# slbouknight/accelerated-ray-tracer

Hardware: AMD Instinct MI355X
Metric: Mrays/s, 1200x800 random scene @ 500 spp (frame ms in ms_per_step) (higher is better)
Workload: dtype f32

## Files before the change

accelerated-ray-tracer_amd/csrc/rt_device_funcs.h:

```cpp
#pragma once
#include <hip/hip_runtime.h>
#include <float.h>
#include <stdint.h>

#include "../../include/rt_abi.h"
#include "rt_device.h"
#include "rt_xorwow.h"

#define DEV __device__ __forceinline__

namespace {

struct f3 { float x, y, z; };
DEV f3 mk3(float x, float y, float z) { f3 r; r.x = x; r.y = y; r.z = z; return r; }
DEV f3 ld3(const float* p) { return mk3(p[0], p[1], p[2]); }
DEV f3 operator+(f3 a, f3 b) { return mk3(a.x + b.x, a.y + b.y, a.z + b.z); }
DEV f3 operator-(f3 a, f3 b) { return mk3(a.x - b.x, a.y - b.y, a.z - b.z); }
DEV f3 operator*(f3 a, f3 b) { return mk3(a.x * b.x, a.y * b.y, a.z * b.z); }
DEV f3 operator*(float t, f3 v) { return mk3(t * v.x, t * v.y, t * v.z); }
DEV f3 operator-(f3 a) { return mk3(-a.x, -a.y, -a.z); }
DEV f3 sdiv(f3 v, float t) { return mk3(v.x / t, v.y / t, v.z / t); }
DEV float dot(f3 a, f3 b) { return fmaf(a.z, b.z, fmaf(a.x, b.x, a.y * b.y)); }
DEV f3 cross(f3 a, f3 b) { return mk3(fmaf(a.y, b.z, -(a.z * b.y)), -fmaf(a.x, b.z, -(a.z * b.x)), fmaf(a.x, b.y, -(a.y * b.x))); }
DEV float length(f3 v) { return sqrtf(fmaf(v.z, v.z, fmaf(v.x, v.x, v.y * v.y))); }
// ... 212 lines not shown
    float t0 = (lo_skip.x - o.x) * inv.x, t1 = (hi_prim.x - o.x) * inv.x;
    if (inv.x < 0.0f) { const float tmp = t0; t0 = t1; t1 = tmp; }
    tmin = t0 > tmin ? t0 : tmin;
    tmax = t1 < tmax ? t1 : tmax;
    t0 = (lo_skip.y - o.y) * inv.y; t1 = (hi_prim.y - o.y) * inv.y;
    if (inv.y < 0.0f) { const float tmp = t0; t0 = t1; t1 = tmp; }
    tmin = t0 > tmin ? t0 : tmin;
    tmax = t1 < tmax ? t1 : tmax;
    t0 = (lo_skip.z - o.z) * inv.z; t1 = (hi_prim.z - o.z) * inv.z;
    if (inv.z < 0.0f) { const float tmp = t0; t0 = t1; t1 = tmp; }
    tmin = t0 > tmin ? t0 : tmin;
    tmax = t1 < tmax ? t1 : tmax;
    return !(tmax <= tmin);
}

DEV void sphere_uv(f3 p, float& u, float& v) {
    const float PI_F = 3.141592654f;
    const float theta = cr_acos(-p.y);
    const float phi = cr_atan2(-p.z, p.x) + PI_F;
    u = phi / (2 * PI_F);
    v = theta / PI_F;
}

template <bool SPHERES_ONLY, bool NEED_UV>
DEV HitRec resolve_hit(const SceneView& sc, const Ray& r, const HitInfo& h) {
    HitRec rec;
    rec.u = 0.f; rec.v = 0.f;
    const int kind = SPHERES_ONLY ? RT_PRIM_SPHERE : RT_PRIM_KIND(h.prim);
    const int idx = RT_PRIM_INDEX(h.prim);
    if (!SPHERES_ONLY && kind == RT_PRIM_MEDIUM) {
        rec.p = ray_at(r, h.t);
        rec.n = mk3(1, 0, 0);
        rec.mat = sc.media[idx].mat;
        return rec;
    }
    Ray q = r;
    rt_instance in;
    const bool through_instance = !SPHERES_ONLY && h.inst >= 0;
    if (through_instance) { in = sc.instances[h.inst]; q = to_object_space(in, r); }
    if (kind == RT_PRIM_SPHERE) {
        const rt_sphere s = sc.spheres[idx];
        const f3 cc = fma3(q.tm, ld3(s.vel), ld3(s.c0));
        rec.p = ray_at(q, h.t);
        rec.n = sdiv(rec.p - cc, s.radius);
        if (NEED_UV && sc.materials[s.mat].pad != 0.0f) sphere_uv(rec.n, rec.u, rec.v);
        rec.mat = s.mat;
    } else {
        const rt_quad qd = sc.quads[idx];
        const f3 P = ray_at(q, h.t);
        const f3 pl = P - ld3(qd.Q);
        const f3 w = ld3(qd.w);
        rec.u = dot(w, cross(pl, ld3(qd.v)));
        rec.v = dot(w, cross(ld3(qd.u), pl));
        f3 n = ld3(qd.n);
        if (dot(n, q.d) > 0.f) n = -n;
        rec.p = P; rec.n = n; rec.mat = qd.mat;
    }
    if (through_instance) {
        if (in.flags & RT_INST_ROTATE_Y) {
            const float c = in.cos_t, s = in.sin_t;
            const float px = fmaf(c, rec.p.x, s * rec.p.z);
            const float pz = fmaf(c, rec.p.z, -(s * rec.p.x));
            const float nx = fmaf(c, rec.n.x, s * rec.n.z);
            const float nz = fmaf(c, rec.n.z, -(s * rec.n.x));
            rec.p = mk3(px, rec.p.y, pz);
            rec.n = unit_vector(mk3(nx, rec.n.y, nz));
            f3 dir_seen = r.d;
            if (dot(rec.n, dir_seen) > 0.f) rec.n = -rec.n;
        }
        if (in.flags & RT_INST_TRANSLATE) rec.p = rec.p + ld3(in.offset);
    }
    return rec;
}

DEV uint32_t wanghash(uint32_t x) {
    x = (x ^ 61u) ^ (x >> 16); x *= 9u; x = x ^ (x >> 4); x *= 0x27d4eb2du; x = x ^ (x >> 15); return x;
}
DEV float u2m11(uint32_t h) { return fmaf((float)((h >> 8) & 0x00FFFFFFu), (1.0f / 8388607.5f), -1.0f); }
DEV f3 perlin_grad(int xi, int yi, int zi) {
    const uint32_t h = wanghash((uint32_t)xi * 73856093u ^ (uint32_t)yi * 19349663u ^ (uint32_t)zi * 83492791u);
    return unit_vector(mk3(u2m11(h), u2m11(wanghash(h)), u2m11(wanghash(h ^ 0x9e3779b9u))));
}
DEV float perlin_noise(f3 p) {
    const float fx = floorf(p.x), fy = floorf(p.y), fz = floorf(p.z);
    const float u = p.x - fx, v = p.y - fy, w = p.z - fz;
    const int i = (int)fx, j = (int)fy, k = (int)fz;
    const float uu = u * u * (3.0f - 2.0f * u), vv = v * v * (3.0f - 2.0f * v), ww = w * w * (3.0f - 2.0f * w);
    float accum = 0.0f;
#pragma unroll
    for (int a = 0; a < 2; ++a)
#pragma unroll
        for (int b = 0; b < 2; ++b)
#pragma unroll
            for (int c = 0; c < 2; ++c) {
                const f3 g = perlin_grad(i + a, j + b, k + c);
                const f3 weight = mk3(u - (float)a, v - (float)b, w - (float)c);
                const float s = (a ? uu : (1.0f - uu)) * (b ? vv : (1.0f - vv)) * (c ? ww : (1.0f - ww));
                accum = fmaf(s, dot(g, weight), accum);
            }
    return accum;
}
__device__ __attribute__((noinline)) float perlin_turb(f3 p, int depth) {
    float accum = 0.0f, weight = 1.0f;
    f3 temp = p;
    for (int i = 0; i < depth; ++i) {
        accum = fmaf(weight, perlin_noise(temp), accum);
        weight *= 0.5f;
        temp = mk3(temp.x * 2.0f, temp.y * 2.0f, temp.z * 2.0f);
    }
    return fabsf(accum);
}

DEV float clamp01(float x) { return x < 0 ? 0 : (x > 1 ? 1 : x); }
template <int TEX>
DEV f3 texture_value(const SceneView& sc, int tex, float u, float v, f3 p) {
    rt_texture t = sc.textures[tex];
    while (t.kind == RT_TEX_CHECKER || (TEX >= 2 && t.kind == RT_TEX_UV_OFFSET)) {
        if (TEX >= 2 && t.kind == RT_TEX_UV_OFFSET) {
            float uu = u + t.scale; uu -= floorf(uu);
            float vv = v + t.p[0]; vv = fminf(fmaxf(vv, 0.f), 1.f);
            u = uu; v = vv;
            t = sc.textures[t.a];
        } else {
            const int xi = (int)floorf(t.scale * p.x);
            const int yi = (int)floorf(t.scale * p.y);
            const int zi = (int)floorf(t.scale * p.z);
            const bool is_even = ((xi + yi + zi) & 1) == 0;
            t = sc.textures[is_even ? t.a : t.b];
        }
    }
    if (TEX < 2 || t.kind == RT_TEX_SOLID) return ld3(t.color);
    if (t.kind == RT_TEX_IMAGE) {
        if (t.a < 0 || t.b <= 0 || t.c <= 0) return mk3(0, 1, 1);
        u = clamp01(u); v = clamp01(v);
        int i = (int)(u * (float)t.b); if (i > t.b - 1) i = t.b - 1;
        int j = (int)((1.f - v) * (float)t.c); if (j > t.c - 1) j = t.c - 1;
        const uint8_t* px = sc.images + (size_t)t.a + (size_t)(j * t.b + i) * 3;
        const float inv255 = 1.f / 255.f;
        return mk3(inv255 * (float)px[0], inv255 * (float)px[1], inv255 * (float)px[2]);
    }
    if (t.kind == RT_TEX_NOODLE) {
        const f3 dir = mk3(t.p[3], t.p[4], t.p[5]);
        const float uu = dot(p, dir);
        const float wig = perlin_turb(t.p[7] * p, t.a);
        const float stripes = fabsf(cr_sin(fmaf(t.scale, uu, t.p[6] * wig)));
        const float q = clamp01((stripes - 0.75f) / (0.98f - 0.75f));
        const float w = q * q * (3.0f - 2.0f * q);
        return fma3(1.f - w, mk3(t.p[0], t.p[1], t.p[2]), w * ld3(t.color));
    }
    if (t.kind == RT_TEX_FELT) {
        const float m = perlin_noise(t.scale * p);
        const float phase = fmaf(p.x, t.p[1], 2.0f * perlin_turb(0.5f * p, 2));
        const float fibers = 0.5f * (1.0f + cr_sin(phase));
        float gain = fmaf(t.p[2], fibers - 0.5f, fmaf(t.p[0], m - 0.5f, 1.0f));
        gain = fminf(fmaxf(gain, 0.7f), 1.2f);
        return gain * ld3(t.color);
    }
    const float s = cr_sin(fmaf(t.scale, p.z, 10.0f * perlin_turb(p, 7)));
    const float g = 0.5f * (1.0f + s);
    return mk3(g, g, g);
}

DEV f3 random_in_unit_sphere(rt_xorwow& g) {
    for (;;) {
        const float a = 2.0f * rt_xorwow_uniform(g) - 1.0f;
        const float b = 2.0f * rt_xorwow_uniform(g) - 1.0f;
        const float c = 2.0f * rt_xorwow_uniform(g) - 1.0f;
        const f3 p = mk3(a, b, c);
        if (dot(p, p) < 1.0f) return p;
    }
}
DEV f3 reflect(f3 v, f3 n) { return fma3(-(2.0f * dot(v, n)), n, v); }
DEV bool refract(f3 v, f3 n, float ni_over_nt, f3& refracted) {
    const f3 uv = unit_vector(v);
    const float dt = dot(uv, n);
    const float disc = fmaf(-(ni_over_nt * ni_over_nt), fmaf(-dt, dt, 1.0f), 1.0f);
    if (disc > 0.0f) {
        refracted = fma3(-sqrtf(disc), n, ni_over_nt * fma3(-dt, n, uv));
        return true;
    }
    return false;
}
DEV float schlick(float cosine, float ref_idx) {
    float r0 = (1.0f - ref_idx) / (1.0f + ref_idx);
    r0 = r0 * r0;
    return fmaf(1.0f - r0, cr_pow5(1.0f - cosine), r0);
}

DEV f3 dielectric_direction(f3 d_in, f3 n, float ior, rt_xorwow& g) {
    f3 outward_normal;
    const f3 reflected = reflect(d_in, n);
    float ni_over_nt, cosine, reflect_prob;
    f3 refracted = mk3(0.f, 0.f, 0.f);
    const float d_n = dot(d_in, n);
    if (d_n > 0.0f) {
        outward_normal = -n;
        ni_over_nt = ior;
        cosine = d_n / length(d_in);
        cosine = sqrtf(fmaxf(0.0f, fmaf(-(ior * ior), fmaf(-cosine, cosine, 1.0f), 1.0f)));
    } else {
        outward_normal = n;
        ni_over_nt = 1.0f / ior;
        cosine = -d_n / length(d_in);
    }
    if (refract(d_in, outward_normal, ni_over_nt, refracted)) reflect_prob = schlick(cosine, ior);
    else reflect_prob = 1.0f;
    return (rt_xorwow_uniform(g) < reflect_prob) ? reflected : refracted;
}

template <int TEX>
DEV bool shade(const SceneView& sc, const Ray& in, const HitRec& rec, rt_xorwow& g, f3& emitted, f3& attenuation, Ray& out) {
    const rt_material m = sc.materials[rec.mat];
    emitted = mk3(0.f, 0.f, 0.f);
    out.o = rec.p;
    out.tm = in.tm;
    switch (m.kind) {
    case RT_MAT_LAMBERTIAN: {
        const f3 target = (rec.p + rec.n) + random_in_unit_sphere(g);
        out.d = target - rec.p;
        attenuation = (TEX > 0 && m.tex >= 0) ? texture_value<TEX>(sc, m.tex, rec.u, rec.v, rec.p) : ld3(m.albedo);
        return true;
    }
    case RT_MAT_METAL: {
        const f3 reflected = reflect(unit_vector(in.d), rec.n);
        const f3 rs = random_in_unit_sphere(g);
        out.d = fma3(m.fuzz, rs, reflected);
        attenuation = ld3(m.albedo);
        return dot(out.d, rec.n) > 0.0f;
    }
    case RT_MAT_DIELECTRIC: {
        attenuation = mk3(1.0f, 1.0f, 1.0f);
        out.d = dielectric_direction(in.d, rec.n, m.ior, g);
        return true;
    }
    case RT_MAT_DIFFUSE_LIGHT: {
        emitted = (TEX > 0 && m.tex >= 0) ? texture_value<TEX>(sc, m.tex, rec.u, rec.v, rec.p) : ld3(m.albedo);
        return false;
    }
    default: {
        out.d = random_in_unit_sphere(g);
        attenuation = (TEX > 0 && m.tex >= 0) ? texture_value<TEX>(sc, m.tex, rec.u, rec.v, rec.p) : ld3(m.albedo);
        return true;
    }
    }
}

DEV Ray camera_get_ray(const rt_camera& c, float s, float t, rt_xorwow& g) {
    f3 p;
    do {
        const float a = rt_xorwow_uniform(g);
        const float b = rt_xorwow_uniform(g);
        p = 2.0f * mk3(a, b, 0.0f) - mk3(1.0f, 1.0f, 0.0f);
    } while (dot(p, p) >= 1.0f);
    const f3 rd = c.lens_radius * p;
    const f3 cu = ld3(c.u), cv = ld3(c.v);
    const f3 offset = fma3(rd.x, cu, rd.y * cv);
    const double tm = fma((double)rt_xorwow_uniform(g), c.time1 - c.time0, c.time0);
    const f3 origin = ld3(c.origin);
    Ray r;
    r.o = origin + offset;
    r.d = (fma3(t, ld3(c.vertical), fma3(s, ld3(c.horizontal), ld3(c.lower_left_corner))) - origin) - offset;
    r.tm = (float)tm;
    return r;
}

DEV float apply_gamma(float c, float gamma) {
    if (gamma == 1.0f) return c;
    const float inv = 1.0f / gamma;
    return cr_pow(fmaxf(c, 0.0f), inv);
}

template <typename P>
DEV f3 miss_color(const P& fp, const Ray& r) {
    f3 bg = mk3(fp.background[0], fp.background[1], fp.background[2]);
    if (fp.use_gradient_bg) {
        const f3 ud = unit_vector(r.d);
        const float t = 0.5f * (ud.y + 1.0f);
        bg = mk3(fmaf(t, 0.5f, 1.0f - t), fmaf(t, 0.7f, 1.0f - t), (1.0f - t) + t);
    }
    return bg;
}

DEV bool work_to_pixel(const rt_frame_params& fp, uint32_t w, int& i, int& lrow) {
    const uint32_t tile = fp.tile_order ? fp.tile_order[w >> 6] : (w >> 6), within = w & 63u;
    const uint32_t tx = tile % (uint32_t)fp.tiles_x, ty = tile / (uint32_t)fp.tiles_x;
    i = (int)(tx * 8u + (within & 7u));
    lrow = (int)(ty * 8u + (within >> 3));
    return i < fp.nx && lrow < fp.local_rows;
}
DEV int local_to_global_row(const rt_frame_params& fp, int lrow) {
    const int t = lrow / fp.tile_rows;
    return (fp.tile_first + t * fp.tile_stride) * fp.tile_rows + (lrow - t * fp.tile_rows);
}

DEV void store_pixel(const rt_frame_params& fp, int i, int lrow, f3 col) {
    const float k = (float)(1.0 / (double)(float)fp.ns);
    col = mk3(col.x * k, col.y * k, col.z * k);
    float* px = fp.fb + ((size_t)lrow * fp.nx + i) * 3;
    px[0] = apply_gamma(col.x, fp.gamma);
    px[1] = apply_gamma(col.y, fp.gamma);
    px[2] = apply_gamma(col.z, fp.gamma);
}

template <int LDS_MODE>
DEV SceneView stage_scene(const rt_scene_dev& sd, unsigned char* lds) {
    SceneView v;
    v.nodes = sd.nodes; v.spheres = sd.spheres; v.quads = sd.quads; v.boxes = sd.boxes; v.instances = sd.instances;
    v.media = sd.media; v.materials = sd.materials; v.textures = sd.textures; v.images = sd.images; v.n_nodes = sd.n_nodes;
    if (LDS_MODE >= 1 && LDS_MODE <= 3) {
        float4* dst = reinterpret_cast<float4*>(lds);
        const float4* src = reinterpret_cast<const float4*>(sd.nodes);
        const int n16 = sd.n_nodes * 2;
        for (int k = threadIdx.x; k < n16; k += blockDim.x) dst[k] = src[k];
        v.nodes = reinterpret_cast<const rt_node*>(lds);
        if (LDS_MODE >= 2) {
            float4* dst2 = dst + n16;
            const float4* src2 = reinterpret_cast<const float4*>(sd.spheres);
            const int m16 = sd.n_spheres * 2;
            for (int k = threadIdx.x; k < m16; k += blockDim.x) dst2[k] = src2[k];
            v.spheres = reinterpret_cast<const rt_sphere*>(dst2);
            if (LDS_MODE >= 3) {
                float4* dst3 = dst2 + m16;
                const float4* src3 = reinterpret_cast<const float4*>(sd.materials);
                const int q16 = sd.n_materials * 2;
                for (int k = threadIdx.x; k < q16; k += blockDim.x) dst3[k] = src3[k];
                v.materials = reinterpret_cast<const rt_material*>(dst3);
                float4* dst4 = dst3 + q16;
                const float4* src4 = reinterpret_cast<const float4*>(sd.textures);
                const int r16 = sd.n_textures * 4;
                for (int k = threadIdx.x; k < r16; k += blockDim.x) dst4[k] = src4[k];
                v.textures = reinterpret_cast<const rt_texture*>(dst4);
            }
        }
        __syncthreads();
    }
    return v;
}

template <bool SPHERES_ONLY>
DEV bool trace(const SceneView& sc, const Ray& r, HitInfo& best, unsigned int* pass_count = nullptr) {
    const f3 inv = mk3(1.0f / r.d.x, 1.0f / r.d.y, 1.0f / r.d.z);
    const float tmin = 0.001f;
    best.t = FLT_MAX; best.prim = -1; best.inst = -1;
    const float4* nodes4 = reinterpret_cast<const float4*>(sc.nodes);
    int i = 0;
    const int n = sc.n_nodes;
    while (i < n) {
        const float4 a = nodes4[2 * i], b = nodes4[2 * i + 1];
        int next = RT_NODE_SKIP(__float_as_int(a.w));
        if (slab_test(a, b, r.o, inv, tmin, best.t)) {
            if (pass_count) atomicAdd(&pass_count[i], 1u);
            const int32_t prim = __float_as_int(b.w);
            if (prim >= 0) leaf_test<SPHERES_ONLY>(sc, prim, r, tmin, best);
            else next = i + 1;
        }
        i = next;
    }
    return best.prim >= 0;
}

DEV bool inv_is_finite(const f3 inv) {
    return fabsf(inv.x) < INFINITY && fabsf(inv.y) < INFINITY && fabsf(inv.z) < INFINITY;
}

DEV void slab_interval(const float4 lo_skip, const float4 hi_prim, const f3 o, const f3 inv, float tmin, float& t_enter, float& t_exit) {
    float tmax = FLT_MAX;
    float t0 = (lo_skip.x - o.x) * inv.x, t1 = (hi_prim.x - o.x) * inv.x;
    if (inv.x < 0.0f) { const float tmp = t0; t0 = t1; t1 = tmp; }
    tmin = t0 > tmin ? t0 : tmin;
    tmax = t1 < tmax ? t1 : tmax;
    t0 = (lo_skip.y - o.y) * inv.y; t1 = (hi_prim.y - o.y) * inv.y;
    if (inv.y < 0.0f) { const float tmp = t0; t0 = t1; t1 = tmp; }
    tmin = t0 > tmin ? t0 : tmin;
    tmax = t1 < tmax ? t1 : tmax;
    t0 = (lo_skip.z - o.z) * inv.z; t1 = (hi_prim.z - o.z) * inv.z;
    if (inv.z < 0.0f) { const float tmp = t0; t0 = t1; t1 = tmp; }
    tmin = t0 > tmin ? t0 : tmin;
    tmax = t1 < tmax ? t1 : tmax;
    t_enter = tmin; t_exit = tmax;
}

DEV bool lane_not(bool b) { return __builtin_amdgcn_inverse_ballot_w64(~__builtin_amdgcn_ballot_w64(b)); }

DEV bool slab_interval_open(float tmin, float tmax, float x0, float x1, float y0, float y1, float z0, float z1) {
    float lo = __builtin_amdgcn_fmed3f(tmin, x0, x1), hi = __builtin_amdgcn_fmed3f(tmax, x0, x1);
    lo = __builtin_amdgcn_fmed3f(lo, y0, y1); hi = __builtin_amdgcn_fmed3f(hi, y0, y1);
    lo = __builtin_amdgcn_fmed3f(lo, z0, z1); hi = __builtin_amdgcn_fmed3f(hi, z0, z1);
    return !(hi <= lo);
}

DEV bool slab_test_finite(const float4 lo_skip, const float4 hi_prim, const f3 o, const f3 inv, float tmin, float tmax) {
    const float x0 = (lo_skip.x - o.x) * inv.x, x1 = (hi_prim.x - o.x) * inv.x;
    const float y0 = (lo_skip.y - o.y) * inv.y, y1 = (hi_prim.y - o.y) * inv.y;
    const float z0 = (lo_skip.z - o.z) * inv.z, z1 = (hi_prim.z - o.z) * inv.z;
    return slab_interval_open(tmin, tmax, x0, x1, y0, y1, z0, z1);
}

struct LooseRay { f3 clo, chi; };
DEV bool loose_ok(const f3 inv, const f3 o, const float* bound) {
    const float ex = fabsf(inv.x) * (fabsf(o.x) + bound[0]), ey = fabsf(inv.y) * (fabsf(o.y) + bound[1]), ez = fabsf(inv.z) * (fabsf(o.z) + bound[2]);
    return fmaxf(fmaxf(ex, ey), ez) < 1e30f;
}
DEV LooseRay loose_setup(const f3 inv, const f3 o, const float* bound) {
    const float k = 9.5367431640625e-07f;
    const float ex = k * (fabsf(inv.x) * (fabsf(o.x) + bound[0])), ey = k * (fabsf(inv.y) * (fabsf(o.y) + bound[1])), ez = k * (fabsf(inv.z) * (fabsf(o.z) + bound[2]));
    const float cx = -(o.x * inv.x), cy = -(o.y * inv.y), cz = -(o.z * inv.z);
    LooseRay r;
    r.clo = mk3(inv.x < 0.0f ? cx + ex : cx - ex, inv.y < 0.0f ? cy + ey : cy - ey, inv.z < 0.0f ? cz + ez : cz - ez);
    r.chi = mk3(inv.x < 0.0f ? cx - ex : cx + ex, inv.y < 0.0f ? cy - ey : cy + ey, inv.z < 0.0f ? cz - ez : cz + ez);
    return r;
}
DEV bool slab_test_loose(const float4 lo_skip, const float4 hi_prim, const f3 inv, const LooseRay& lr, float tmin, float tmax) {
    const float x0 = fmaf(lo_skip.x, inv.x, lr.clo.x), x1 = fmaf(hi_prim.x, inv.x, lr.chi.x);
    const float y0 = fmaf(lo_skip.y, inv.y, lr.clo.y), y1 = fmaf(hi_prim.y, inv.y, lr.chi.y);
    const float z0 = fmaf(lo_skip.z, inv.z, lr.clo.z), z1 = fmaf(hi_prim.z, inv.z, lr.chi.z);
    return slab_interval_open(tmin, tmax, x0, x1, y0, y1, z0, z1);
}

}
```

accelerated-ray-tracer_amd/csrc/rt_kernel_staged.h:

```cpp
#pragma once
#ifndef RT_STEP_UNROLL
#define RT_STEP_UNROLL 2
#endif
#include "rt_device_funcs.h"
#include "rt_launch.h"

#ifdef RT_DIAG
#define DIAG_ADD(slot, value) do { const unsigned long long v_ = (unsigned long long)(value); if ((threadIdx.x & 63) == 0) diag_local[slot] += v_; } while (0)
#define DIAG_T(slot) do { const unsigned long long n_ = __builtin_readcyclecounter(); diag_time[slot] += n_ - diag_t_last; diag_t_last = n_; } while (0)
#else
#define DIAG_ADD(slot, value) do { } while (0)
#define DIAG_T(slot) do { } while (0)
#endif

template <bool SPHERES_ONLY, int TEX, bool NEED_UV, int LDS_MODE>
__global__ void __launch_bounds__((SPHERES_ONLY && TEX < 2) ? RT_LEAN_MAX_THREADS : RT_HEAVY_MAX_THREADS, (SPHERES_ONLY && TEX < 2) ? RT_LEAN_MIN_WAVES : RT_HEAVY_MIN_WAVES) rt_render_staged_kernel(rt_scene_dev sd, rt_frame_params fp) {
    extern __shared__ __attribute__((aligned(16))) unsigned char lds[];
#ifdef RT_DIAG
    unsigned long long diag_local[16] = {0, 0, 0, 0, 0, 0, 0, 0, 0, 0, 0, 0, 0, 0, 0, 0};
    unsigned long long diag_time[8] = {0, 0, 0, 0, 0, 0, 0, 0};
    unsigned long long diag_shade_cycles = 0;
    unsigned long long diag_t_last = 0;
    const unsigned long long diag_t_start = __builtin_amdgcn_s_memrealtime();
    if ((threadIdx.x & 63) == 0) atomicMin(fp.ray_counter + RT_DIAG_T0_SLOT, diag_t_start);
    unsigned long long diag_fetch_t = 0ull, diag_done_t = 0ull;
    unsigned int diag_last_px = 0u, diag_last_src = 0u;
#endif
    constexpr bool SCAN = LDS_MODE == 4;
    rt_rank_info rk;
    rk.heavy_items = 0u; rk.heavy_threshold = 0xFFFFFFFFu; rk.tier1_items = 0u; rk.tier2_items = 0u;
    rk.tier1_wgs = 0; rk.main_skip_wgs = 0; rk.sparse_wgs = 0; rk.sparse_stride = 1; rk.semi_wgs = 0; rk.semi_stride = 1;
    if (fp.rank) {
        const rt_rank_info* q = fp.rank;
        rk.heavy_items = q->heavy_items; rk.heavy_threshold = q->heavy_threshold; rk.tier1_items = q->tier1_items;
        rk.tier2_items = q->tier2_items; rk.semi_wgs = q->semi_wgs; rk.semi_stride = q->semi_stride;
        rk.main_skip_wgs = q->main_skip_wgs; rk.sparse_wgs = q->sparse_wgs; rk.sparse_stride = q->sparse_stride;
    }
    const int wg = (int)blockIdx.x - rk.main_skip_wgs;
    if (wg < 0) return;
    const SceneView sc = stage_scene<LDS_MODE>(sd, lds);
    const float4* nodes4 = reinterpret_cast<const float4*>(sc.nodes);
    const int n_nodes = sc.n_nodes;
    const int ST_DONE = n_nodes, ST_NEWPATH = n_nodes + 1, ST_DIEL = n_nodes + 2, ST_SETUP = n_nodes + 3, ST_DEAD = n_nodes + 4;
    const float tmin = 0.001f;

    rt_xorwow g = {0, 0, 0, 0, 0, 0};
    int px_i = 0, px_lrow = 0, px_j = 0, sample = 0, bounce = 0;
    f3 col = mk3(0, 0, 0), throughput = mk3(1, 1, 1), radiance = mk3(0, 0, 0);
    Ray cur; cur.o = mk3(0, 0, 0); cur.d = mk3(0, 0, 1); cur.tm = 0.f;
    f3 inv = mk3(1, 1, 1);
    HitInfo best; best.t = FLT_MAX; best.prim = -1; best.inst = -1;
    int node = ST_NEWPATH;
    int32_t parked = -1;
    int32_t pend = -1;
    float cur_a = 1.f;
    bool have_pixel = false, first = true, finite_inv = true;
    bool tier3_open = true;
    bool leave = false;
    unsigned int wave_dead = 0;
    unsigned long long last_poll = 0ull;
    bool dry_seen = false;
    const uint32_t total_lanes = (uint32_t)((int)gridDim.x - rk.main_skip_wgs) * blockDim.x;
    unsigned int rays = 0, rays_at_pixel_start = 0;
    bool sparse = wg < rk.sparse_wgs;
    bool semi = !sparse && wg < rk.sparse_wgs + rk.semi_wgs;
#ifdef RT_DIAG
    const bool diag_was_sparse = sparse;
#endif
    if (semi && fp.semi_priority > 0) {
        if (fp.semi_priority == 1) __builtin_amdgcn_s_setprio(1);
        else if (fp.semi_priority == 2) __builtin_amdgcn_s_setprio(2);
        else __builtin_amdgcn_s_setprio(3);
    }
    if (sparse && fp.sparse_priority > 0) {
        if (fp.sparse_priority == 1) __builtin_amdgcn_s_setprio(1);
        else if (fp.sparse_priority == 2) __builtin_amdgcn_s_setprio(2);
        else __builtin_amdgcn_s_setprio(3);
    }

#ifdef RT_DIAG
    diag_t_last = __builtin_readcyclecounter();
#endif
    for (;;) {
        DIAG_ADD(0, 1);
        DIAG_T(7);
        if (SCAN) {
            const bool scanning = (unsigned)node < (unsigned)n_nodes;
            if (__ballot(scanning) != 0ull) {
                const bool ref_form = __ballot(scanning && !finite_inv) != 0ull;
                int resume = 0;
                for (int k = 0; k < n_nodes; ++k) {
                    const float4 a = uniform_load(nodes4 + 2 * k), b = uniform_load(nodes4 + 2 * k + 1);
                    const int32_t prim = __builtin_amdgcn_readfirstlane(__float_as_int(b.w));
                    const int skip = RT_NODE_SKIP(__builtin_amdgcn_readfirstlane(__float_as_int(a.w)));
                    const bool active = scanning && k >= resume;
                    DIAG_ADD(1, 1); DIAG_ADD(2, __popcll(__ballot(active)));
                    const bool pass = active && (ref_form ? slab_test(a, b, cur.o, inv, tmin, best.t) : slab_test_finite(a, b, cur.o, inv, tmin, best.t));
                    if (prim < 0) {
                        if (active && !pass) resume = skip;
                        DIAG_T(0);
                    } else if (__ballot(pass) != 0ull) {
                        DIAG_T(0);
                        DIAG_ADD(3, 1); DIAG_ADD(4, __popcll(__ballot(pass)));
                        if (pass) leaf_test<SPHERES_ONLY, true>(sc, prim, cur, tmin, best);
                        DIAG_T(1);
                    }
                }
                if (scanning) node = ST_DONE;
            }
        } else {
        if (__ballot(!finite_inv && (unsigned)node < (unsigned)n_nodes) == 0ull) {
            const int trip_pairs = ((sparse ? 2 * fp.steps_per_trip : fp.steps_per_trip) + RT_STEP_UNROLL - 1) / RT_STEP_UNROLL;
            const LooseRay lr = loose_setup(inv, cur.o, sd.bound);
            for (int pair = 0; pair < trip_pairs; ++pair) {
                if (__ballot((unsigned)node < (unsigned)n_nodes) == 0ull) break;
#pragma unroll
                for (int half = 0; half < RT_STEP_UNROLL; ++half) {
                    DIAG_ADD(1, 1); DIAG_ADD(2, __popcll(__ballot((unsigned)node < (unsigned)n_nodes)));
                    if ((unsigned)node < (unsigned)n_nodes) {
                        const float4 a = nodes4[2 * node], b = nodes4[2 * node + 1];
                        const bool pass = slab_test_loose(a, b, inv, lr, tmin, best.t);
                        const int32_t link = __float_as_int(b.w), nskip = __float_as_int(a.w);
                        const bool is_leaf = link >= 0, noted = pend >= 0;
                        const bool inner = lane_not(is_leaf), clear = lane_not(noted);
                        const bool at_leaf = pass && is_leaf;
                        const bool stop = at_leaf && noted;
                        const int next = ~((pass && inner) ? link : nskip);
                        pend = (at_leaf && clear) ? node : pend;
                        parked = stop ? node : parked;
                        node = stop ? nskip : next;
                    }
                }
            }
        } else {
            for (int step = 0; step < fp.steps_per_trip; ++step) {
                if (__ballot((unsigned)node < (unsigned)n_nodes) == 0ull) break;
                if ((unsigned)node < (unsigned)n_nodes) {
                    const float4 a = nodes4[2 * node], b = nodes4[2 * node + 1];
                    const bool pass = slab_test(a, b, cur.o, inv, tmin, best.t);
                    const int32_t link = __float_as_int(b.w), nskip = __float_as_int(a.w);
                    const bool at_leaf = pass && link >= 0;
                    const bool stop = at_leaf && (pend >= 0 || !finite_inv);
                    const int next = ~((pass && link < 0) ? link : nskip);
                    pend = (at_leaf && !stop) ? node : pend;
                    parked = stop ? node : parked;
                    node = stop ? nskip : next;
                }
            }
        }
        DIAG_T(0);
        for (;;) {
            const int cand = pend >= 0 ? pend : (node < 0 ? parked : -1);
            const unsigned long long due_mask = __ballot(cand >= 0);
            const bool nobody_steps = __ballot((unsigned)node < (unsigned)n_nodes) == 0ull;
            const int live_b = __popcll(__ballot(node != ST_DEAD));
            if (due_mask != 0ull && (nobody_steps || sparse || __popcll(due_mask) >= 1 + ((fp.leaf_threshold - 1) * live_b >> 6))) {
                DIAG_ADD(3, 1); DIAG_ADD(4, __popcll(due_mask));
                int kind = -1;
                int32_t prim = -1;
                bool box_ok = false;
                if (cand >= 0) {
                    const float4 a = nodes4[2 * cand], b = nodes4[2 * cand + 1];
                    prim = __float_as_int(b.w);
                    kind = SPHERES_ONLY ? RT_PRIM_SPHERE : RT_PRIM_KIND(prim);
                    box_ok = finite_inv ? slab_test_finite(a, b, cur.o, inv, tmin, best.t) : true;
                }
                bool tested = false;
                if (SPHERES_ONLY) {
                    if (cand >= 0) {
                        float t;
                        if (box_ok && sphere_test_a(sc.spheres[RT_PRIM_INDEX(prim)], cur, cur_a, tmin, best.t, t)) { best.t = t; best.prim = prim; best.inst = -1; }
                        tested = true;
                    }
                } else {
                    if (kind == RT_PRIM_SPHERE || kind == RT_PRIM_QUAD) {
                        float t;
                        const bool hit = box_ok && (kind == RT_PRIM_SPHERE ? sphere_test_a(sc.spheres[RT_PRIM_INDEX(prim)], cur, cur_a, tmin, best.t, t)
                                                                           : quad_test(sc.quads[RT_PRIM_INDEX(prim)], cur, tmin, best.t, t));
                        if (hit) { best.t = t; best.prim = prim; best.inst = -1; }
                        tested = true;
                    }
                    const unsigned long long box_mask = __ballot(kind == RT_PRIM_BOX || kind == RT_PRIM_INSTANCE);
                    if (box_mask != 0ull && (nobody_steps || __popcll(box_mask) >= 1 + ((fp.box_threshold - 1) * live_b >> 6))) {
                        if (kind == RT_PRIM_BOX || kind == RT_PRIM_INSTANCE) {
                            float t;
                            int32_t leaf = prim, inst = -1;
                            if (box_ok && solid_test(sc, prim, cur, tmin, best.t, t, leaf, inst)) { best.t = t; best.prim = leaf; best.inst = inst; }
                            tested = true;
                        }
                    }
                    const unsigned long long med_mask = __ballot(kind == RT_PRIM_MEDIUM);
                    if (med_mask != 0ull && (nobody_steps || __popcll(med_mask) >= 1 + ((fp.medium_threshold - 1) * live_b >> 6))) {
                        if (kind == RT_PRIM_MEDIUM) {
                            float t;
                            if (box_ok && medium_test(sc, sc.media[RT_PRIM_INDEX(prim)], cur, tmin, best.t, t)) { best.t = t; best.prim = prim; best.inst = -1; }
                            tested = true;
                        }
                    }
                }
                if (tested) {
                    if (node < 0) { pend = pend >= 0 ? parked : -1; parked = -1; node = ~node; }
                    else pend = -1;
                }
                if (nobody_steps && __ballot((unsigned)node < (unsigned)n_nodes) == 0ull && __ballot(pend >= 0 || node < 0) != 0ull) continue;
            }
            break;
        }
        }
        DIAG_T(1);
        if (node == ST_DONE && pend < 0 && best.prim < 0) {
            radiance = fma3(throughput, miss_color(fp, cur), radiance);
            node = ST_NEWPATH;
        }
        const unsigned long long walking = __ballot(node < n_nodes);
        const bool force = walking == 0ull;
        const int n_done = __popcll(__ballot(node == ST_DONE && pend < 0));
        bool ran_stage = false;
        const int live = __popcll(__ballot(node != ST_DEAD));
        const int shade_need = 1 + ((fp.shade_threshold - 1) * live >> 6);
        const int diel_need = 1 + ((fp.diel_threshold - 1) * live >> 6);
        const int newpath_need = 1 + ((fp.newpath_threshold - 1) * live >> 6);
        const bool eager = sparse && fp.sparse_eager;

        DIAG_T(6);
        if (n_done > 0 && (n_done >= shade_need || force || eager)) {
            ran_stage = true;
            DIAG_ADD(5, 1); DIAG_ADD(6, n_done);
            DIAG_ADD(11, __popcll(__ballot(node == ST_DONE && pend < 0 && best.prim >= 0)));
            if (node == ST_DONE && pend < 0) {
                {
                    const HitRec rec = resolve_hit<SPHERES_ONLY, NEED_UV>(sc, cur, best);
                    const rt_material m = sc.materials[rec.mat];
                    if (m.kind == RT_MAT_DIELECTRIC) {
                        if (sparse) {
                            const f3 dir = dielectric_direction(cur.d, rec.n, m.ior, g);
                            ++bounce;
                            if (bounce >= 50) node = ST_NEWPATH;
                            else { cur.o = rec.p; cur.d = dir; node = ST_SETUP; }
                        } else {
                            node = ST_DIEL;
                        }
                    } else if (m.kind == RT_MAT_DIFFUSE_LIGHT) {
                        const f3 emitted = (TEX > 0 && m.tex >= 0) ? texture_value<TEX>(sc, m.tex, rec.u, rec.v, rec.p) : ld3(m.albedo);
                        radiance = fma3(throughput, emitted, radiance);
                        node = ST_NEWPATH;
                    } else {
                        const f3 rs = random_in_unit_sphere(g);
                        f3 dir, attenuation;
                        bool go_on = true;
                        if (m.kind == RT_MAT_METAL) {
                            const f3 reflected = reflect(unit_vector(cur.d), rec.n);
                            dir = fma3(m.fuzz, rs, reflected);
                            attenuation = ld3(m.albedo);
                            go_on = dot(dir, rec.n) > 0.0f;
                        } else {
                            if (m.kind == RT_MAT_LAMBERTIAN) {
                                const f3 target = (rec.p + rec.n) + rs;
                                dir = target - rec.p;
                            } else {
                                dir = rs;
                            }
                            attenuation = (TEX > 0 && m.tex >= 0) ? texture_value<TEX>(sc, m.tex, rec.u, rec.v, rec.p) : ld3(m.albedo);
                        }
                        ++bounce;
                        if (!go_on || bounce >= 50) node = ST_NEWPATH;
                        else {
                            throughput = throughput * attenuation;
                            cur.o = rec.p; cur.d = dir;
                            node = ST_SETUP;
                        }
                    }
                }
            }
        }
        DIAG_T(2);
        {
            const int n_diel = __popcll(__ballot(node == ST_DIEL));
            if (n_diel > 0 && (n_diel >= diel_need || force || eager)) {
                ran_stage = true;
                DIAG_ADD(7, 1); DIAG_ADD(8, n_diel);
                if (node == ST_DIEL) {
                    const HitRec rec = resolve_hit<SPHERES_ONLY, false>(sc, cur, best);
                    const f3 dir = dielectric_direction(cur.d, rec.n, sc.materials[rec.mat].ior, g);
                    ++bounce;
                    if (bounce >= 50) node = ST_NEWPATH;
                    else { throughput = throughput * mk3(1.0f, 1.0f, 1.0f); cur.o = rec.p; cur.d = dir; node = ST_SETUP; }
                }
            }
        }
        DIAG_T(3);
        {
            const int n_new = __popcll(__ballot(node == ST_NEWPATH));
            if (n_new > 0 && (n_new >= newpath_need || force || eager)) {
                ran_stage = true;
                DIAG_ADD(9, 1); DIAG_ADD(10, n_new);
                if (fp.handoff_queue && !leave && dry_seen) {
                    const unsigned long long now = __builtin_amdgcn_s_memrealtime();
                    if (now - last_poll >= (unsigned long long)fp.handoff_poll_ticks) {
                        last_poll = now;
                        const uint32_t dead = __hip_atomic_load(fp.work_counter + RT_WC_DEAD, __ATOMIC_RELAXED, __HIP_MEMORY_SCOPE_AGENT);
                        leave = __builtin_amdgcn_readfirstlane((int)(total_lanes - dead)) <= fp.handoff_pixels;
                    }
                }
                bool ran_dry = false;
                if (node == ST_NEWPATH) {
                    if (!first) { col = col + radiance; ++sample; }
                    first = false;
                    bool alive = true;
                    const bool part_done = sample >= fp.sample_end;
                    bool hand = have_pixel && !part_done && leave;
                    uint32_t slot = 0u;
                    if (hand) { slot = atomicAdd(fp.work_counter + RT_WC_PUSHED, 1u); hand = slot < fp.handoff_cap; }
                    if (have_pixel && (part_done || hand)) {
                        if (fp.state_out || hand) {
                            const unsigned int c = rays - rays_at_pixel_start;
                            const size_t at = (size_t)px_lrow * fp.nx + px_i;
                            rt_pixel_state st;
                            st.rng[0] = g.v0; st.rng[1] = g.v1; st.rng[2] = g.v2; st.rng[3] = g.v3; st.rng[4] = g.v4; st.rng[5] = g.d;
                            st.col[0] = col.x; st.col[1] = col.y; st.col[2] = col.z;
                            st.cost = c + (fp.state_in ? (fp.fresh ? (fp.state_in[at].cost & 0x80000000u) : fp.state_in[at].cost) : 0u);
                            (hand ? fp.handoff_state : fp.state_out)[at] = st;
                            if (fp.tile_cost) atomicAdd(&fp.tile_cost[(px_lrow >> 3) * fp.tiles_x + (px_i >> 3)], c);
                            if (hand) {
                                fp.handoff_queue[slot] = ((unsigned long long)(uint32_t)sample << 32) | (unsigned long long)at;
                                alive = false;
                            } else if (fp.store_parked) store_pixel(fp, px_i, px_lrow, col);
                        } else {
                            store_pixel(fp, px_i, px_lrow, col);
                            if (fp.cost_out) {
                                const size_t at = (size_t)px_lrow * fp.nx + px_i;
                                fp.cost_out[at] = ((rays - rays_at_pixel_start) + ((fp.state_in && !fp.fresh) ? fp.state_in[at].cost : 0u)) & 0x7FFFFFFFu;
                            }
                        }
                        have_pixel = false;
                    }
                    while (!have_pixel && alive) {
                        bool ok;
                        if (sparse) {
                            if (((threadIdx.x & 63) % (unsigned)rk.sparse_stride) != 0u) { alive = false; break; }
                            const uint32_t k2 = atomicAdd(fp.work_counter + 1, 1u);
                            if (k2 >= rk.tier2_items) { alive = false; ran_dry = true; break; }
                            const uint32_t at = rk.tier1_items + k2;
                            const uint32_t pix = fp.heavy_pixels[at];
                            px_lrow = (int)(pix / (uint32_t)fp.nx); px_i = (int)(pix - (uint32_t)px_lrow * (uint32_t)fp.nx);
                            ok = true;
                        } else if (tier3_open && (semi || rk.semi_wgs == 0)) {
                            if (semi && ((threadIdx.x & 63) % (unsigned)rk.semi_stride) != 0u) { alive = false; break; }
                            const uint32_t k3 = atomicAdd(fp.work_counter + 4, 1u);
                            const uint32_t first3 = rk.tier1_items + rk.tier2_items;
                            if (first3 + k3 >= rk.heavy_items) { tier3_open = false; if (semi) { alive = false; ran_dry = true; break; } continue; }
                            const uint32_t pix = fp.heavy_pixels[first3 + k3];
                            px_lrow = (int)(pix / (uint32_t)fp.nx); px_i = (int)(pix - (uint32_t)px_lrow * (uint32_t)fp.nx);
                            ok = true;
                        } else {
                            const uint32_t w = atomicAdd(fp.work_counter, 1u);
                            if (w >= fp.work_items) { alive = false; ran_dry = true; break; }
                            ok = work_to_pixel(fp, w, px_i, px_lrow);
                            if (ok && rk.heavy_items && (fp.state_in[(size_t)px_lrow * fp.nx + px_i].cost & 0x80000000u) != 0u) ok = false;
                        }
                        if (ok) {
#ifdef RT_DIAG
                            diag_fetch_t = __builtin_amdgcn_s_memrealtime(); diag_last_px = (unsigned int)px_lrow * (unsigned int)fp.nx + (unsigned int)px_i;
                            diag_last_src = sparse ? 2u : (tier3_open ? 3u : 0u);
#endif
                            px_j = local_to_global_row(fp, px_lrow);
                            if (fp.state_in && !fp.fresh) {
                                const rt_pixel_state st = fp.state_in[(size_t)px_lrow * fp.nx + px_i];
                                g.v0 = st.rng[0]; g.v1 = st.rng[1]; g.v2 = st.rng[2]; g.v3 = st.rng[3]; g.v4 = st.rng[4]; g.d = st.rng[5];
                                col = mk3(st.col[0], st.col[1], st.col[2]);
                            } else {
                                rt_xorwow_seed(g, fp.seed_base + (uint64_t)(px_j * fp.nx + px_i));
                                col = mk3(0, 0, 0);
                            }
                            sample = fp.sample_begin; have_pixel = true;
                            rays_at_pixel_start = rays;
                        }
                    }
                    if (alive) {
                        const float u = ((float)px_i + rt_xorwow_uniform(g)) / (float)fp.nx;
                        const float v = ((float)px_j + rt_xorwow_uniform(g)) / (float)fp.ny;
                        cur = camera_get_ray(sd.camera, u, v, g);
                        throughput = mk3(1, 1, 1); radiance = mk3(0, 0, 0); bounce = 0;
                        node = ST_SETUP;
                    } else {
                        node = ST_DEAD;
#ifdef RT_DIAG
                        diag_done_t = __builtin_amdgcn_s_memrealtime();
#endif
                    }
                }
                if (fp.handoff_queue) {
                    dry_seen = dry_seen || __ballot(ran_dry) != 0ull;
                    const unsigned int n_died = (unsigned int)__popcll(__ballot(node == ST_DEAD));
                    if (n_died != wave_dead) {
                        if ((threadIdx.x & 63) == 0) atomicAdd(fp.work_counter + RT_WC_DEAD, n_died - wave_dead);
                        wave_dead = n_died;
                    }
                }
            }
        }
        DIAG_T(4);
        if (ran_stage) {
            DIAG_ADD(12, 1); DIAG_ADD(13, __popcll(__ballot(node == ST_SETUP)));
            if (node == ST_SETUP) {
                inv = mk3(1.0f / cur.d.x, 1.0f / cur.d.y, 1.0f / cur.d.z);
                finite_inv = inv_is_finite(inv) && loose_ok(inv, cur.o, sd.bound);
                cur_a = dot(cur.d, cur.d);
                best.t = FLT_MAX; best.prim = -1; best.inst = -1;
                node = n_nodes > 0 ? 0 : ST_DONE;
                ++rays;
            }
        } else if (force) {
            if (!sparse && !semi) break;
            sparse = false; semi = false;
            if (fp.handoff_queue && wave_dead) {
                if ((threadIdx.x & 63) == 0) atomicAdd(fp.work_counter + RT_WC_DEAD, 0u - wave_dead);
                wave_dead = 0;
            }
            __builtin_amdgcn_s_setprio(0);
            node = ST_NEWPATH; first = true; have_pixel = false;
        }
    }
    unsigned long long r64 = rays;
    for (int off = 32; off > 0; off >>= 1) r64 += __shfl_down(r64, off, 64);
    if ((threadIdx.x & 63) == 0 && r64) atomicAdd(fp.ray_counter, r64);
#ifdef RT_DIAG
    if ((threadIdx.x & 63) == 0) {
        for (int k = 0; k < 16; ++k) atomicAdd(fp.ray_counter + 1 + k, diag_local[k]);
        for (int k = 0; k < 8; ++k) atomicAdd(fp.ray_counter + 17 + k, diag_time[k]);
        if (diag_shade_cycles) atomicAdd(fp.ray_counter + 25, diag_shade_cycles);
        const unsigned long long t0 = *reinterpret_cast<volatile unsigned long long*>(fp.ray_counter + RT_DIAG_T0_SLOT);
        const unsigned long long now = __builtin_amdgcn_s_memrealtime();
        unsigned long long bin = now > t0 ? (now - t0) / 100000ull : 0ull;
        if (bin >= (unsigned long long)RT_DIAG_BINS) bin = RT_DIAG_BINS - 1;
        atomicAdd(fp.ray_counter + RT_DIAG_HIST_SLOT + (diag_was_sparse ? RT_DIAG_BINS : 0) + bin, 1ull);
    }
    {
        unsigned long long best_done = diag_done_t;
        for (int off = 32; off > 0; off >>= 1) { const unsigned long long o = __shfl_xor(best_done, off, 64); best_done = o > best_done ? o : best_done; }
        const unsigned long long t0 = *reinterpret_cast<volatile unsigned long long*>(fp.ray_counter + RT_DIAG_T0_SLOT);
        const unsigned int wave_id = blockIdx.x * (blockDim.x >> 6) + (threadIdx.x >> 6);
        if (diag_done_t == best_done && best_done != 0ull && wave_id < (unsigned int)RT_DIAG_MAX_WAVES) {
            const unsigned long long f_us = diag_fetch_t > t0 ? (diag_fetch_t - t0) / 100ull : 0ull, d_us = best_done > t0 ? (best_done - t0) / 100ull : 0ull;
            fp.ray_counter[RT_DIAG_WAVE_SLOT + 2 * wave_id] = (d_us << 32) | (f_us & 0xFFFFFFFFull);
            fp.ray_counter[RT_DIAG_WAVE_SLOT + 2 * wave_id + 1] = ((unsigned long long)diag_last_src << 60) | ((unsigned long long)(diag_was_sparse ? 1u : 0u) << 59) | diag_last_px;
        }
    }
#endif
}

template <bool SO, int TX, bool UV>
static hipError_t rt_launch_staged_family(int lds_mode, const rt_scene_dev& sd, const rt_frame_params& fp, dim3 grid, dim3 block,
                                          size_t lds, hipStream_t st) {
    if (lds_mode == 4) return rt_launch_kernel(rt_render_staged_kernel<SO, TX, UV, 4>, block, grid, lds, st, sd, fp);
    if (lds_mode == 3) return rt_launch_kernel(rt_render_staged_kernel<SO, TX, UV, 3>, block, grid, lds, st, sd, fp);
    if (lds_mode == 2) return rt_launch_kernel(rt_render_staged_kernel<SO, TX, UV, 2>, block, grid, lds, st, sd, fp);
    if (lds_mode == 1) return rt_launch_kernel(rt_render_staged_kernel<SO, TX, UV, 1>, block, grid, lds, st, sd, fp);
    return rt_launch_kernel(rt_render_staged_kernel<SO, TX, UV, 0>, block, grid, lds, st, sd, fp);
}
```

Before: 13470.

## Store BVH links as precomputed LDS byte addresses during node staging

When nodes are staged into LDS, the skip/child link fields are rewritten into absolute LDS byte addresses, and leaf primitive indices are stored complemented. The traversal loop then uses node addresses directly as its state, which removes the index-to-address multiply/add and the bitwise-not per step. Node state sentinels are shifted so they sit past the LDS address range. This adds a rewrite pass during staging and relies on the precise encoding conventions for leaf, skip and parked nodes. The parked-node resume now reads the skip word back from LDS.

```diff
diff --git a/accelerated-ray-tracer_amd/csrc/rt_device_funcs.h b/accelerated-ray-tracer_amd/csrc/rt_device_funcs.h
--- a/accelerated-ray-tracer_amd/csrc/rt_device_funcs.h
+++ b/accelerated-ray-tracer_amd/csrc/rt_device_funcs.h
@@ -538,7 +538,15 @@
     px[2] = apply_gamma(col.z, fp.gamma);
 }
 
-template <int LDS_MODE>
+typedef float lds_native_float4 __attribute__((ext_vector_type(4)));
+DEV int32_t lds_address(const void* p) { return (int32_t)(uint32_t)(uintptr_t)(const __attribute__((address_space(3))) void*)p; }
+DEV float4 lds_load_float4(int32_t address, int which) {
+    const lds_native_float4 q = ((const __attribute__((address_space(3))) lds_native_float4*)(uintptr_t)(uint32_t)address)[which];
+    return make_float4(q.x, q.y, q.z, q.w);
+}
+DEV int32_t lds_load_word(int32_t address, int word) { return ((const __attribute__((address_space(3))) int32_t*)(uintptr_t)(uint32_t)address)[word]; }
+
+template <int LDS_MODE, bool WALK_LINKS = false>
 DEV SceneView stage_scene(const rt_scene_dev& sd, unsigned char* lds) {
     SceneView v;
     v.nodes = sd.nodes; v.spheres = sd.spheres; v.quads = sd.quads; v.boxes = sd.boxes; v.instances = sd.instances;
@@ -547,7 +555,17 @@
         float4* dst = reinterpret_cast<float4*>(lds);
         const float4* src = reinterpret_cast<const float4*>(sd.nodes);
         const int n16 = sd.n_nodes * 2;
-        for (int k = threadIdx.x; k < n16; k += blockDim.x) dst[k] = src[k];
+        if (WALK_LINKS) {
+            const int32_t base = lds_address(lds);
+            for (int k = threadIdx.x; k < n16; k += blockDim.x) {
+                float4 q = src[k];
+                const int32_t w = __float_as_int(q.w);
+                q.w = __int_as_float(w < 0 ? base + 32 * RT_NODE_SKIP(w) : ~w);
+                dst[k] = q;
+            }
+        } else {
+            for (int k = threadIdx.x; k < n16; k += blockDim.x) dst[k] = src[k];
+        }
         v.nodes = reinterpret_cast<const rt_node*>(lds);
         if (LDS_MODE >= 2) {
             float4* dst2 = dst + n16;
diff --git a/accelerated-ray-tracer_amd/csrc/rt_kernel_staged.h b/accelerated-ray-tracer_amd/csrc/rt_kernel_staged.h
--- a/accelerated-ray-tracer_amd/csrc/rt_kernel_staged.h
+++ b/accelerated-ray-tracer_amd/csrc/rt_kernel_staged.h
@@ -38,10 +38,16 @@
     }
     const int wg = (int)blockIdx.x - rk.main_skip_wgs;
     if (wg < 0) return;
-    const SceneView sc = stage_scene<LDS_MODE>(sd, lds);
+    constexpr bool ADDR = LDS_MODE >= 1 && LDS_MODE <= 3;
+    const SceneView sc = stage_scene<LDS_MODE, ADDR>(sd, lds);
     const float4* nodes4 = reinterpret_cast<const float4*>(sc.nodes);
     const int n_nodes = sc.n_nodes;
-    const int ST_DONE = n_nodes, ST_NEWPATH = n_nodes + 1, ST_DIEL = n_nodes + 2, ST_SETUP = n_nodes + 3, ST_DEAD = n_nodes + 4;
+    const int root = ADDR ? lds_address(lds) : 0;
+    const int limit = ADDR ? __builtin_amdgcn_readfirstlane(root + 32 * n_nodes) : n_nodes;
+    const int ST_DONE = limit, ST_NEWPATH = limit + 1, ST_DIEL = limit + 2, ST_SETUP = limit + 3, ST_DEAD = limit + 4;
+    auto node_lo = [&](int at) -> float4 { return ADDR ? lds_load_float4(at, 0) : nodes4[2 * at]; };
+    auto node_hi = [&](int at) -> float4 { return ADDR ? lds_load_float4(at, 1) : nodes4[2 * at + 1]; };
+    auto leaf_prim = [](const float4 hi) -> int32_t { return ADDR ? ~__float_as_int(hi.w) : __float_as_int(hi.w); };
     const float tmin = 0.001f;
 
     rt_xorwow g = {0, 0, 0, 0, 0, 0};
@@ -109,42 +115,62 @@
                 if (scanning) node = ST_DONE;
             }
         } else {
-        if (__ballot(!finite_inv && (unsigned)node < (unsigned)n_nodes) == 0ull) {
+        if (__ballot(!finite_inv && (unsigned)node < (unsigned)limit) == 0ull) {
             const int trip_pairs = ((sparse ? 2 * fp.steps_per_trip : fp.steps_per_trip) + RT_STEP_UNROLL - 1) / RT_STEP_UNROLL;
             const LooseRay lr = loose_setup(inv, cur.o, sd.bound);
             for (int pair = 0; pair < trip_pairs; ++pair) {
-                if (__ballot((unsigned)node < (unsigned)n_nodes) == 0ull) break;
+                if (__ballot((unsigned)node < (unsigned)limit) == 0ull) break;
 #pragma unroll
                 for (int half = 0; half < RT_STEP_UNROLL; ++half) {
-                    DIAG_ADD(1, 1); DIAG_ADD(2, __popcll(__ballot((unsigned)node < (unsigned)n_nodes)));
-                    if ((unsigned)node < (unsigned)n_nodes) {
-                        const float4 a = nodes4[2 * node], b = nodes4[2 * node + 1];
+                    DIAG_ADD(1, 1); DIAG_ADD(2, __popcll(__ballot((unsigned)node < (unsigned)limit)));
+                    if ((unsigned)node < (unsigned)limit) {
+                        const float4 a = node_lo(node), b = node_hi(node);
                         const bool pass = slab_test_loose(a, b, inv, lr, tmin, best.t);
+                        if (ADDR) {
+                            const int32_t link = __float_as_int(b.w), skip = __float_as_int(a.w);
+                            const bool is_leaf = link < 0, noted = pend >= 0;
+                            const bool inner = lane_not(is_leaf), clear = lane_not(noted);
+                            const bool at_leaf = pass && is_leaf;
+                            const bool stop = at_leaf && noted;
+                            pend = (at_leaf && clear) ? node : pend;
+                            parked = stop ? node : parked;
+                            node = (pass && (inner || noted)) ? link : skip;
+                        } else {
+                            const int32_t link = __float_as_int(b.w), nskip = __float_as_int(a.w);
+                            const bool is_leaf = link >= 0, noted = pend >= 0;
+                            const bool inner = lane_not(is_leaf), clear = lane_not(noted);
+                            const bool at_leaf = pass && is_leaf;
+                            const bool stop = at_leaf && noted;
+                            const int next = ~((pass && inner) ? link : nskip);
+                            pend = (at_leaf && clear) ? node : pend;
+                            parked = stop ? node : parked;
+                            node = stop ? nskip : next;
+                        }
+                    }
+                }
+            }
+        } else {
+            for (int step = 0; step < fp.steps_per_trip; ++step) {
+                if (__ballot((unsigned)node < (unsigned)limit) == 0ull) break;
+                if ((unsigned)node < (unsigned)limit) {
+                    const float4 a = node_lo(node), b = node_hi(node);
+                    const bool pass = slab_test(a, b, cur.o, inv, tmin, best.t);
+                    if (ADDR) {
+                        const int32_t link = __float_as_int(b.w), skip = __float_as_int(a.w);
+                        const bool at_leaf = pass && link < 0;
+                        const bool stop = at_leaf && (pend >= 0 || !finite_inv);
+                        pend = (at_leaf && !stop) ? node : pend;
+                        parked = stop ? node : parked;
+                        node = (pass && (link >= 0 || stop)) ? link : skip;
+                    } else {
                         const int32_t link = __float_as_int(b.w), nskip = __float_as_int(a.w);
-                        const bool is_leaf = link >= 0, noted = pend >= 0;
-                        const bool inner = lane_not(is_leaf), clear = lane_not(noted);
-                        const bool at_leaf = pass && is_leaf;
-                        const bool stop = at_leaf && noted;
-                        const int next = ~((pass && inner) ? link : nskip);
-                        pend = (at_leaf && clear) ? node : pend;
+                        const bool at_leaf = pass && link >= 0;
+                        const bool stop = at_leaf && (pend >= 0 || !finite_inv);
+                        const int next = ~((pass && link < 0) ? link : nskip);
+                        pend = (at_leaf && !stop) ? node : pend;
                         parked = stop ? node : parked;
                         node = stop ? nskip : next;
                     }
-                }
-            }
-        } else {
-            for (int step = 0; step < fp.steps_per_trip; ++step) {
-                if (__ballot((unsigned)node < (unsigned)n_nodes) == 0ull) break;
-                if ((unsigned)node < (unsigned)n_nodes) {
-                    const float4 a = nodes4[2 * node], b = nodes4[2 * node + 1];
-                    const bool pass = slab_test(a, b, cur.o, inv, tmin, best.t);
-                    const int32_t link = __float_as_int(b.w), nskip = __float_as_int(a.w);
-                    const bool at_leaf = pass && link >= 0;
-                    const bool stop = at_leaf && (pend >= 0 || !finite_inv);
-                    const int next = ~((pass && link < 0) ? link : nskip);
-                    pend = (at_leaf && !stop) ? node : pend;
-                    parked = stop ? node : parked;
-                    node = stop ? nskip : next;
                 }
             }
         }
@@ -152,7 +178,7 @@
         for (;;) {
             const int cand = pend >= 0 ? pend : (node < 0 ? parked : -1);
             const unsigned long long due_mask = __ballot(cand >= 0);
-            const bool nobody_steps = __ballot((unsigned)node < (unsigned)n_nodes) == 0ull;
+            const bool nobody_steps = __ballot((unsigned)node < (unsigned)limit) == 0ull;
             const int live_b = __popcll(__ballot(node != ST_DEAD));
             if (due_mask != 0ull && (nobody_steps || sparse || __popcll(due_mask) >= 1 + ((fp.leaf_threshold - 1) * live_b >> 6))) {
                 DIAG_ADD(3, 1); DIAG_ADD(4, __popcll(due_mask));
@@ -160,8 +186,8 @@
                 int32_t prim = -1;
                 bool box_ok = false;
                 if (cand >= 0) {
-                    const float4 a = nodes4[2 * cand], b = nodes4[2 * cand + 1];
-                    prim = __float_as_int(b.w);
+                    const float4 a = node_lo(cand), b = node_hi(cand);
+                    prim = leaf_prim(b);
                     kind = SPHERES_ONLY ? RT_PRIM_SPHERE : RT_PRIM_KIND(prim);
                     box_ok = finite_inv ? slab_test_finite(a, b, cur.o, inv, tmin, best.t) : true;
                 }
@@ -199,10 +225,13 @@
                     }
                 }
                 if (tested) {
-                    if (node < 0) { pend = pend >= 0 ? parked : -1; parked = -1; node = ~node; }
+                    if (node < 0) {
+                        node = ADDR ? lds_load_word(parked, 3) : ~node;
+                        pend = pend >= 0 ? parked : -1; parked = -1;
+                    }
                     else pend = -1;
                 }
-                if (nobody_steps && __ballot((unsigned)node < (unsigned)n_nodes) == 0ull && __ballot(pend >= 0 || node < 0) != 0ull) continue;
+                if (nobody_steps && __ballot((unsigned)node < (unsigned)limit) == 0ull && __ballot(pend >= 0 || node < 0) != 0ull) continue;
             }
             break;
         }
@@ -212,7 +241,7 @@
             radiance = fma3(throughput, miss_color(fp, cur), radiance);
             node = ST_NEWPATH;
         }
-        const unsigned long long walking = __ballot(node < n_nodes);
+        const unsigned long long walking = __ballot(node < limit);
         const bool force = walking == 0ull;
         const int n_done = __popcll(__ballot(node == ST_DONE && pend < 0));
         bool ran_stage = false;
@@ -407,7 +436,7 @@
                 finite_inv = inv_is_finite(inv) && loose_ok(inv, cur.o, sd.bound);
                 cur_a = dot(cur.d, cur.d);
                 best.t = FLT_MAX; best.prim = -1; best.inst = -1;
-                node = n_nodes > 0 ? 0 : ST_DONE;
+                node = n_nodes > 0 ? root : ST_DONE;
                 ++rays;
             }
         } else if (force) {
```

Result: faster. 13980, median of 6 (+3.7%).
